# adityabalu/DiffNet

Hardware: AMD Instinct MI355X
Metric: elements*gauss_pts/sec (FEM loss+grad) (higher is better)
Workload: dtype f32; 1 GPU; 2-D Poisson energy loss + gradient wrt u, Q1, 512^2 nodes, 3^2 Gauss pts, batch 64/GPU, nu+f nodal fields, Dirichlet mask on all boundary faces held as one bit per node and sample (a general mask array), fused single pass (BASELINE.json configs[1] mesh); every step evaluates the next of 4 different batches in rotation (nu, f and the mask stream from HBM with non-temporal loads; of the 4 x 67 MB of; batch_per_gpu=64, parallelism=batch-sharded x1, batches_in_rotation=4, mask_format=bits

## Files before the change

### diffnet_amd/csrc/poisson2d_q1_cf.hip

```cpp
#include <cstdlib>
#include <type_traits>

#define DN_NT_STORES 1
#include "poisson_common.h"

namespace dn {

enum : int { CF_NU = 1, CF_F = 2, CF_BC = 8, CF_BC_U8C = 16, CF_BC_PACKED = 32, CF_PK_NB1 = 64, CF_PK_NB2 = 128, CF_UA = 256 };

template <int E>
struct CfRow {
    float u[E + 1], n[E + 1], f[E + 1];
    float g[E + 1];
    float keep[E];
    float keepx;
    BcRaw<E> bc;
    uint32_t m8[2][2];
    uint32_t mb[2];
    uint32_t bx[2];
};

constexpr int CF_W = 4;
constexpr int CF_TS = 128;
constexpr int CF_NSLOT = 64;
constexpr unsigned CF_SPIN_MAX = 1u << 20;

__device__ __forceinline__ unsigned lds_addr(const void* p) { return (unsigned)(uintptr_t)(__attribute__((address_space(3))) const void*)p; }
__device__ __forceinline__ void lds_st(unsigned a, float v) { asm volatile("ds_write_b32 %0, %1" ::"v"(a), "v"(v) : "memory"); }
__device__ __forceinline__ void lds_st(unsigned a, unsigned v) { asm volatile("ds_write_b32 %0, %1" ::"v"(a), "v"(v) : "memory"); }
__device__ __forceinline__ void lds_ld_nowait(float& d, unsigned a) { asm volatile("ds_read_b32 %0, %1" : "=v"(d) : "v"(a) : "memory"); }
__device__ __forceinline__ unsigned lds_ld_u(unsigned a) {
    unsigned d;
    asm volatile("ds_read_b32 %0, %1\n\ts_waitcnt lgkmcnt(0)" : "=v"(d) : "v"(a) : "memory");
    return d;
}
__device__ __forceinline__ float lds_ld(unsigned a) {
    float d;
    asm volatile("ds_read_b32 %0, %1\n\ts_waitcnt lgkmcnt(0)" : "=v"(d) : "v"(a) : "memory");
    return d;
}
template <int N>
__device__ __forceinline__ void lds_wait(float (&v)[N]) {
    if constexpr (N == 5) asm volatile("s_waitcnt lgkmcnt(0)" : "+v"(v[0]), "+v"(v[1]), "+v"(v[2]), "+v"(v[3]), "+v"(v[4])::"memory");
    else if constexpr (N == 4) asm volatile("s_waitcnt lgkmcnt(0)" : "+v"(v[0]), "+v"(v[1]), "+v"(v[2]), "+v"(v[3])::"memory");
    else if constexpr (N == 3) asm volatile("s_waitcnt lgkmcnt(0)" : "+v"(v[0]), "+v"(v[1]), "+v"(v[2])::"memory");
    else if constexpr (N == 2) asm volatile("s_waitcnt lgkmcnt(0)" : "+v"(v[0]), "+v"(v[1])::"memory");
    else { static_assert(N == 1, "lds_wait: 1..5 values"); asm volatile("s_waitcnt lgkmcnt(0)" : "+v"(v[0])::"memory"); }
}

template <int E, bool VEC, int FL, int W>
__global__ void __launch_bounds__(W > 1 ? CF_TS * W : 256, W > 1 ? 4 : 2) poisson2d_q1_cf_kernel(const PoissonParams p) {
    constexpr int NW = E;
    constexpr bool HAS_NU = (FL & CF_NU) != 0, HAS_F = (FL & CF_F) != 0;
    constexpr bool BC_ANY = (FL & (CF_BC | CF_BC_U8C | CF_BC_PACKED)) != 0, BC_U8C = (FL & CF_BC_U8C) != 0, BC_PACKED = (FL & CF_BC_PACKED) != 0;
    constexpr bool UA = (FL & CF_UA) != 0;
    static_assert(!UA || (E == 4 && VEC && W == 1), "CF_UA: four elements per thread, vector accesses, one strip per workgroup");
    const int T = W > 1 ? CF_TS : (int)blockDim.x;
    const int sub = W > 1 ? __builtin_amdgcn_readfirstlane((int)threadIdx.x / CF_TS) : 0;
    const int tid = W > 1 ? (int)threadIdx.x - sub * CF_TS : (int)threadIdx.x;
    const int chunk = blockIdx.x, strip = W > 1 ? (int)blockIdx.y * W + sub : selected_strip(p, (int)blockIdx.y), b = blockIdx.z;
    const bool active = W == 1 || strip < p.nstrips;
    const bool chain_dn = W > 1 && sub > 0;
    const bool chain_up = W > 1 && sub + 1 < W && strip + 1 < p.nstrips;
    const int q = chunk * (T - 1) + tid;
    const int ex0 = q * E;
    const int x0 = ex0;
    const bool col_owner = !(chunk > 0 && tid == 0);
    const bool lastcol = UA && x0 + NW == p.nx - 1;
    const int64_t nps = (int64_t)p.nx * p.ny;
    const SampleBases sb = sample_bases(p, b, nps);
    const int R = p.rows_per_strip;
    const int sb0 = strip * R, sc0 = min(sb0 + R, p.nely);
    const int ey_begin = (sb0 > 0 && !chain_dn) ? sb0 - 1 : sb0;
    const int ey_end = sc0;
    const int r_from = sb0;
    const int e_from = sb0, e_until = p.nely;
    const bool top_row = sc0 == p.nely;

    __shared__ float xch[2][256];
    __shared__ double red[W > 1 ? 4 * W : 8];
    __shared__ int last_flag;
    constexpr int CW = W > 1 ? W : 2, SEAM_WORDS = 6 * (E + 1);
    __shared__ float cf_edge[W > 1 ? W : 1][W > 1 ? CF_NSLOT : 1];
    __shared__ unsigned cf_xflag[W > 1 ? W : 1];
    __shared__ float cf_seam[CW - 1][W > 1 ? SEAM_WORDS : 1][W > 1 ? CF_TS : 1];
    __shared__ unsigned cf_sflag[CW - 1][2][2];
    const int lane = tid & 63, wv = __builtin_amdgcn_readfirstlane(tid >> 6);
    unsigned seq = 0u;
    if constexpr (W > 1) {
        static_assert(CF_TS == 128, "two waves per sub-strip");
        if (threadIdx.x < (unsigned)W) cf_xflag[threadIdx.x] = 0u;
        if (threadIdx.x < 4u * (W - 1)) (&cf_sflag[0][0][0])[threadIdx.x] = 0u;
        __syncthreads();
    }
    if ((blockIdx.x | blockIdx.y | blockIdx.z) == 0u) fold_prev_sums(p, (int)threadIdx.x, (int)blockDim.x, red);
    float spin_poison = 0.f;
    auto spin_until = [&](const unsigned* flag, unsigned want) {
        const unsigned fa = lds_addr(flag);
        const unsigned lim = p.spin_limit > 0 ? (unsigned)p.spin_limit : CF_SPIN_MAX;
        unsigned n = 0;
        for (; n < lim; ++n) {
            if ((unsigned)__builtin_amdgcn_readfirstlane((int)lds_ld_u(fa)) >= want) break;
            __builtin_amdgcn_s_sleep(1);
        }
        if (n == lim) spin_poison = __builtin_nanf("");
    };

    const bool has_mask[2] = {sb.mask[0] != nullptr, sb.mask[1] != nullptr};
    const uint8_t* mask8[2];
    mask8[0] = reinterpret_cast<const uint8_t*>(has_mask[0] ? sb.mask[0] : sb.mask[1]);
    mask8[1] = reinterpret_cast<const uint8_t*>(has_mask[1] ? sb.mask[1] : sb.mask[0]);

    constexpr unsigned NBITS = (1u << (NW + 1)) - 1u;
    constexpr int NB = !BC_PACKED ? 0 : ((FL & CF_PK_NB2) ? 2 : ((FL & CF_PK_NB1) ? 1 : 0));
    const bool isbits[2] = {p.bc[0].kind == DN_MASK_BITS, p.bc[1].kind == DN_MASK_BITS};
    const unsigned bsel[2] = {isbits[0] ? NBITS : 0u, isbits[1] ? NBITS : 0u};
    const int src0 = (NB == 2 || isbits[0]) ? 0 : 1;
    const uint32_t* bptr[2] = {reinterpret_cast<const uint32_t*>(sb.mask[src0]), reinterpret_cast<const uint32_t*>(sb.mask[1])};
    const unsigned brow[2] = {(unsigned)p.bc[src0].row_bytes / 4u, (unsigned)p.bc[1].row_bytes / 4u};
    unsigned bw0[2], bw1[2];
#pragma unroll
    for (int j = 0; j < 2; ++j) {
        const int rw = max((int)brow[j], 1);
        bw0[j] = (unsigned)min(x0 >> 5, rw - 1);
        bw1[j] = (unsigned)min((x0 >> 5) + 1, rw - 1);
    }
    const unsigned bsh = (unsigned)x0 & 31u;
    unsigned boxx[2] = {0u, 0u};
#pragma unroll
    for (int k = 0; k < 2; ++k) {
        const int faces = p.bc[k].kind == DN_MASK_BOX ? p.bc[k].box_faces : 0;
#pragma unroll
        for (int n = 0; n <= NW; ++n) {
            const bool on = ((faces & DN_FACE_XLO) && x0 + n == 0) || ((faces & DN_FACE_XHI) && x0 + n == p.nx - 1);
            boxx[k] |= on ? (1u << n) : 0u;
        }
    }
    const int ylo[2] = {(p.bc[0].kind == DN_MASK_BOX && (p.bc[0].box_faces & DN_FACE_YLO)) ? 0 : -1,
                        (p.bc[1].kind == DN_MASK_BOX && (p.bc[1].box_faces & DN_FACE_YLO)) ? 0 : -1};
    const int yhi[2] = {(p.bc[0].kind == DN_MASK_BOX && (p.bc[0].box_faces & DN_FACE_YHI)) ? p.ny - 1 : -1,
                        (p.bc[1].kind == DN_MASK_BOX && (p.bc[1].box_faces & DN_FACE_YHI)) ? p.ny - 1 : -1};
    auto packed_issue = [&](int yc, CfRow<E>& r) {
#pragma unroll
        for (int j = 0; j < NB; ++j) {
            const unsigned ro = (unsigned)yc * brow[j];
            const uint32_t w0 = ld_at<uint32_t>(bptr[j], ro + bw0[j]), w1 = ld_at<uint32_t>(bptr[j], ro + bw1[j]);
            r.mb[j] = __builtin_amdgcn_alignbit(w1, w0, bsh);
        }
#pragma unroll
        for (int k = 0; k < 2; ++k) r.bx[k] = (yc == ylo[k] || yc == yhi[k]) ? NBITS : boxx[k];
    };

    auto row_issue = [&](int yr, CfRow<E>& r) {
        const int yp = min(yr, p.ny - 1);
        const unsigned rowoff = (unsigned)yp * (unsigned)p.nx;
        load_seg<NW, VEC>(sb.u, rowoff, x0, p.nx, r.u);
        if constexpr (HAS_NU) load_seg_stream<NW, VEC>(sb.nu, rowoff, x0, p.nx, r.n);
        if constexpr (HAS_F) load_seg_stream<NW, VEC>(sb.f, rowoff, x0, p.nx, r.f);
        if constexpr (BC_PACKED) {
            packed_issue(yp, r);
        } else if constexpr (BC_U8C) {
#pragma unroll
            for (int k = 0; k < 2; ++k) {
                if (has_mask[k]) {
                    uint8_t t[NW + 1];
                    load_seg_stream<NW, VEC>(mask8[k], rowoff, x0, p.nx, t);
                    uint32_t w = 0u;
#pragma unroll
                    for (int n = 0; n < NW; ++n) w |= (uint32_t)t[n] << (8 * n);
                    r.m8[k][0] = w;
                    r.m8[k][1] = t[NW];
                }
            }
        } else if constexpr (BC_ANY) {
            bc_issue<NW, VEC>(p, sb, rowoff, x0, r.bc);
        }
    };
    auto row_bc = [&](CfRow<E>& r) {
#pragma unroll
        for (int n = 0; n < NW; ++n) r.keep[n] = 1.f;
        if constexpr (UA) r.keepx = 1.f;
        if constexpr (BC_PACKED) {
            unsigned b0 = r.bx[0], b1 = r.bx[1];
            if constexpr (NB == 2) { b0 |= r.mb[0] & bsel[0]; b1 |= r.mb[1] & bsel[1]; }
            if constexpr (NB == 1) { b0 |= r.mb[0] & bsel[0]; b1 |= r.mb[0] & bsel[1]; }
            const float v0 = p.bc[0].value, v1 = p.bc[1].value;
#pragma unroll
            for (int n = 0; n <= NW; ++n) {
                r.u[n] = (b0 & (1u << n)) ? v0 : r.u[n];
                r.u[n] = (b1 & (1u << n)) ? v1 : r.u[n];
                if (n < NW) r.keep[n] = ((b0 | b1) & (1u << n)) ? 0.f : 1.f;
            }
            if constexpr (UA) r.keepx = ((b0 | b1) & (1u << NW)) ? 0.f : 1.f;
        } else if constexpr (BC_U8C) {
#pragma unroll
            for (int k = 0; k < 2; ++k) {
                if (has_mask[k]) {
                    const float val = p.bc[k].value;
#pragma unroll
                    for (int n = 0; n <= NW; ++n) {
                        const bool set = has_mask[k] && (n < NW ? ((r.m8[k][0] >> (8 * n)) & 0xffu) != 0u : r.m8[k][1] != 0u);
                        r.u[n] = set ? val : r.u[n];
                        if (n < NW) r.keep[n] = set ? 0.f : r.keep[n];
                        else if constexpr (UA) r.keepx = set ? 0.f : r.keepx;
                    }
                }
            }
        } else if constexpr (BC_ANY) {
            if constexpr (UA) {
                float k5[NW + 1];
                bc_apply_all<NW>(p, sb, r.bc, r.u, k5);
#pragma unroll
                for (int n = 0; n < NW; ++n) r.keep[n] = k5[n];
                r.keepx = k5[NW];
            } else {
                bc_apply<NW>(p, sb, r.bc, r.u, r.keep);
            }
        }
    };

    float e1_acc = 0.f, e2_acc = 0.f, sq_acc = 0.f;
    int par = 0;

    float pend_v[NW];
    unsigned pend_row = 0u;
    bool pend_st = false;
    float pend_x = 0.f;
    auto flush_store = [&]() {
        if (pend_st) store_seg<NW, VEC>(sb.out, pend_row, x0, p.nx, pend_v);
        if constexpr (UA) {
            if (pend_st && lastcol) st_at<float>(sb.out, pend_row + (unsigned)(p.nx - 1), pend_x);
        }
        pend_st = false;
    };
    auto emit_row = [&](const float (&o)[NW + 1], const float (&keep)[NW], int yr, bool owned_row, float keepx = 1.f) {
        float left;
        if constexpr (W > 1) {
            const float up = __shfl_up(o[NW], 1, 64);
            const unsigned ea = lds_addr(&cf_edge[sub][seq & (CF_NSLOT - 1)]);
            float edge = 0.f;
            if (wv == 0) {
                if (lane == 63) { lds_st(ea, o[NW]); lds_st(lds_addr(&cf_xflag[sub]), seq + 1u); }
            } else {
                spin_until(&cf_xflag[sub], seq + 1u);
                edge = lds_ld(ea);
            }
            left = lane > 0 ? up : edge;
            ++seq;
        } else {
            xch[par][tid] = o[NW];
            asm volatile("s_waitcnt lgkmcnt(0)\n\ts_barrier" ::: "memory");
            left = (tid > 0) ? xch[par][tid - 1] : 0.f;
            par ^= 1;
        }
        const bool st = owned_row && col_owner && (!UA || x0 + NW <= p.nx - 1);
#pragma unroll
        for (int n = 0; n < NW; ++n) {
            const float t = (o[n] + (n == 0 ? left : 0.f)) * keep[n];
            sq_acc = st ? fmaf(t, t, sq_acc) : sq_acc;
            pend_v[n] = t * p.out_scale;
            if constexpr (W > 1) pend_v[n] += spin_poison;
        }
        if constexpr (UA) {
            const float t = o[NW] * keepx;
            sq_acc = (st && lastcol) ? fmaf(t, t, sq_acc) : sq_acc;
            pend_x = t * p.out_scale;
        }
        pend_row = (unsigned)yr * (unsigned)p.nx;
        pend_st = st && sb.out != nullptr;
        flush_store();
    };

    const float mx0 = p.T.mxs[0], mx1 = p.T.mxs[1], mx2 = p.T.mxs[2], mx3 = p.T.mxs[3];
    const float my0 = p.T.m[0], my1 = p.T.m[1], my2 = p.T.m[2], my3 = p.T.m[3];
    const float k0 = p.T.q1c[0], k1 = p.T.q1c[1], h0 = p.T.q1c[2], h1 = p.T.q1c[3], nb = -p.T.beta;

    constexpr bool FMASS = HAS_F && (FL & CF_BC) == 0;
    const float cx00 = p.T.q1mx[0], cx01 = p.T.q1mx[1], cx11 = p.T.q1mx[2], cy00 = p.T.q1my[0], cy01 = p.T.q1my[1], cy11 = p.T.q1my[2];
    auto fstage = [&](CfRow<E>& r) {
        if constexpr (FMASS) {
#pragma unroll
            for (int n = 0; n <= NW; ++n) r.g[n] = 0.f;
#pragma unroll
            for (int e = 0; e < E; ++e) {
                if (ex0 + e < p.nelx) {
                    r.g[e] = fmaf(cx01, r.f[e + 1], fmaf(cx00, r.f[e], r.g[e]));
                    r.g[e + 1] = fmaf(cx11, r.f[e + 1], cx01 * r.f[e]);
                }
            }
        }
    };

    auto layer = [&](auto fresh, int ey, const CfRow<E>& L, CfRow<E>& U, const float (&cin)[NW + 1], float (&cout)[NW + 1]) {
        const bool own_layer = ey >= e_from && ey <= e_until;
        const float cnt = (own_layer && col_owner) ? 1.f : 0.f;
        if constexpr (decltype(fresh)::value) { row_bc(U); fstage(U); }
        float o[NW + 1], le1 = 0.f, le2 = 0.f;
#pragma unroll
        for (int n = 0; n <= NW; ++n) { o[n] = cin[n]; cout[n] = 0.f; }
        if constexpr (FMASS) {
#pragma unroll
            for (int n = 0; n <= NW; ++n) {
                const float tlo = fmaf(cy01, U.g[n], cy00 * L.g[n]), tup = fmaf(cy11, U.g[n], cy01 * L.g[n]);
                o[n] = fmaf(nb, tlo, o[n]);
                cout[n] = nb * tup;
                le2 = fmaf(U.u[n], tup, fmaf(L.u[n], tlo, le2));
            }
        }
#pragma unroll
        for (int e = 0; e < E; ++e) {
            if (ex0 + e < p.nelx) {
                const float U0 = L.u[e], UX = L.u[e + 1] - L.u[e], UY = U.u[e] - L.u[e], UXY = (U.u[e + 1] - U.u[e]) - UX;
                float P = mx0, Q = 0.f, Pp = my0, Qp = 0.f;
                if constexpr (HAS_NU) {
                    const float N0 = L.n[e], NX = L.n[e + 1] - N0, NY = U.n[e] - N0, NXY = (U.n[e + 1] - U.n[e]) - NX;
                    P = fmaf(mx1, NX, mx0 * N0);
                    Q = fmaf(mx1, NXY, mx0 * NY);
                    Pp = fmaf(my1, NY, my0 * N0);
                    Qp = fmaf(my1, NXY, my0 * NX);
                }
                const float A0 = fmaf(Q, my1, P * my0), A1 = fmaf(Q, my2, P * my1), A2 = fmaf(Q, my3, P * my2);
                const float B0 = fmaf(Qp, mx1, Pp * mx0), B1 = fmaf(Qp, mx2, Pp * mx1), B2 = fmaf(Qp, mx3, Pp * mx2);
                const float tX0 = fmaf(UXY, A1, UX * A0), tX1 = fmaf(UXY, A2, UX * A1);
                const float tY0 = fmaf(UXY, B1, UY * B0), tY1 = fmaf(UXY, B2, UY * B1);
                le1 += fmaf(h1, fmaf(UXY, tY1, UY * tY0), h0 * fmaf(UXY, tX1, UX * tX0));
                float cU0 = 0.f, cUX = k0 * tX0, cUY = k1 * tY0, cUXY = fmaf(k0, tX1, k1 * tY1);
                if constexpr (HAS_F && !FMASS) {
                    const float F0 = L.f[e], FX = L.f[e + 1] - F0, FY = U.f[e] - F0, FXY = (U.f[e + 1] - U.f[e]) - FX;
                    const float S0 = fmaf(mx1, FX, mx0 * F0), S1 = fmaf(mx1, FXY, mx0 * FY);
                    const float T0 = fmaf(mx2, FX, mx1 * F0), T1 = fmaf(mx2, FXY, mx1 * FY);
                    const float L0 = fmaf(my1, S1, my0 * S0), LX = fmaf(my1, T1, my0 * T0);
                    const float LY = fmaf(my2, S1, my1 * S0), LXY = fmaf(my2, T1, my1 * T0);
                    le2 += fmaf(LXY, UXY, fmaf(LY, UY, fmaf(LX, UX, L0 * U0)));
                    cU0 = nb * L0;
                    cUX = fmaf(nb, LX, cUX);
                    cUY = fmaf(nb, LY, cUY);
                    cUXY = fmaf(nb, LXY, cUXY);
                }
                const float g01 = cUX - cUXY, g10 = cUY - cUXY;
                o[e] += (cU0 - cUX) - g10;
                o[e + 1] += g01;
                cout[e] += g10;
                cout[e + 1] += cUXY;
            }
        }
        e1_acc = fmaf(cnt, le1, e1_acc);
        e2_acc = fmaf(cnt, le2, e2_acc);
        if (W > 1 && chain_dn && ey == sb0) {
            const unsigned s0 = lds_addr(&cf_seam[W > 1 ? sub - 1 : 0][0][tid]);
#pragma unroll
            for (int n = 0; n <= NW; ++n) lds_st(s0 + (4 * NW + 4 + n) * CF_TS * 4, o[n]);
#pragma unroll
            for (int n = 0; n < NW; ++n) lds_st(s0 + (5 * NW + 5 + n) * CF_TS * 4, L.keep[n]);
        } else {
            emit_row(o, L.keep, ey, ey >= r_from, L.keepx);
        }
    };
    auto publish_row = [&](const CfRow<E>& r) {
        const unsigned s0 = lds_addr(&cf_seam[W > 1 ? sub - 1 : 0][0][tid]);
#pragma unroll
        for (int n = 0; n <= NW; ++n) {
            lds_st(s0 + n * CF_TS * 4, r.u[n]);
            if constexpr (HAS_NU) lds_st(s0 + (NW + 1 + n) * CF_TS * 4, r.n[n]);
            if constexpr (FMASS) lds_st(s0 + (2 * NW + 2 + n) * CF_TS * 4, r.g[n]);
            else if constexpr (HAS_F) lds_st(s0 + (2 * NW + 2 + n) * CF_TS * 4, r.f[n]);
        }
        if (lane == 0) lds_st(lds_addr(&cf_sflag[W > 1 ? sub - 1 : 0][0][wv]), 1u);
    };
    auto fetch_row = [&](CfRow<E>& r) {
        spin_until(&cf_sflag[sub][0][wv], 1u);
        const unsigned s0 = lds_addr(&cf_seam[sub][0][tid]);
#pragma unroll
        for (int n = 0; n <= NW; ++n) lds_ld_nowait(r.u[n], s0 + n * CF_TS * 4);
        lds_wait(r.u);
        if constexpr (HAS_NU) {
#pragma unroll
            for (int n = 0; n <= NW; ++n) lds_ld_nowait(r.n[n], s0 + (NW + 1 + n) * CF_TS * 4);
            lds_wait(r.n);
        }
        if constexpr (FMASS) {
#pragma unroll
            for (int n = 0; n <= NW; ++n) lds_ld_nowait(r.g[n], s0 + (2 * NW + 2 + n) * CF_TS * 4);
            lds_wait(r.g);
        } else if constexpr (HAS_F) {
#pragma unroll
            for (int n = 0; n <= NW; ++n) lds_ld_nowait(r.f[n], s0 + (2 * NW + 2 + n) * CF_TS * 4);
            lds_wait(r.f);
        }
    };
    auto publish_carry = [&](const float (&c)[NW + 1]) {
        const unsigned s0 = lds_addr(&cf_seam[sub][0][tid]);
#pragma unroll
        for (int n = 0; n <= NW; ++n) lds_st(s0 + (3 * NW + 3 + n) * CF_TS * 4, c[n]);
        if (lane == 0) lds_st(lds_addr(&cf_sflag[sub][1][wv]), 1u);
    };

    auto set_prio = [&](int e) {
        switch (((ey_end - e) >> 1) & 3) {
            case 0: __builtin_amdgcn_s_setprio(0); break;
            case 1: __builtin_amdgcn_s_setprio(1); break;
            case 2: __builtin_amdgcn_s_setprio(2); break;
            default: __builtin_amdgcn_s_setprio(3); break;
        }
    };

    constexpr std::true_type FRESH{};
    constexpr std::false_type LANDED{};
    if (active) {
    CfRow<E> RA, RB;
    float carryA[NW + 1], carryB[NW + 1];
#pragma unroll
    for (int n = 0; n <= NW; ++n) carryA[n] = carryB[n] = 0.f;
    row_issue(ey_begin, RA);
    row_bc(RA);
    fstage(RA);
    if constexpr (W > 1) {
        if (chain_dn) publish_row(RA);
    }
    int ey = ey_begin;
    bool odd = false;
    const int n_main = chain_up ? ey_end - 1 : ey_end;
    for (; ey + 1 < n_main; ey += 2) {
        set_prio(ey);
        row_issue(ey + 1, RB);
        layer(FRESH, ey, RA, RB, carryA, carryB);
        row_issue(ey + 2, RA);
        layer(FRESH, ey + 1, RB, RA, carryB, carryA);
    }
    if (ey < n_main) {
        set_prio(ey);
        row_issue(ey + 1, RB);
        layer(FRESH, ey, RA, RB, carryA, carryB);
        odd = true;
        ++ey;
    }
    if constexpr (W > 1) {
        if (chain_up) {
            __builtin_amdgcn_s_setprio(0);
            if (odd) { fetch_row(RA); layer(LANDED, ey, RB, RA, carryB, carryA); publish_carry(carryA); }
            else { fetch_row(RB); layer(LANDED, ey, RA, RB, carryA, carryB); publish_carry(carryB); }
        }
    }
    if (top_row) {
        float o[NW + 1], keep[NW];
#pragma unroll
        for (int n = 0; n <= NW; ++n) o[n] = odd ? carryB[n] : carryA[n];
#pragma unroll
        for (int n = 0; n < NW; ++n) keep[n] = odd ? RB.keep[n] : RA.keep[n];
        emit_row(o, keep, p.ny - 1, true, odd ? RB.keepx : RA.keepx);
        flush_store();
    }
    if constexpr (W > 1) {
        if (chain_dn) {
            spin_until(&cf_sflag[sub - 1][1][wv], 1u);
            const unsigned s0 = lds_addr(&cf_seam[sub - 1][0][tid]);
            float o[NW + 1], cy[NW + 1], keep[NW];
#pragma unroll
            for (int n = 0; n <= NW; ++n) lds_ld_nowait(o[n], s0 + (4 * NW + 4 + n) * CF_TS * 4);
            lds_wait(o);
#pragma unroll
            for (int n = 0; n <= NW; ++n) lds_ld_nowait(cy[n], s0 + (3 * NW + 3 + n) * CF_TS * 4);
            lds_wait(cy);
#pragma unroll
            for (int n = 0; n < NW; ++n) lds_ld_nowait(keep[n], s0 + (5 * NW + 5 + n) * CF_TS * 4);
            lds_wait(keep);
#pragma unroll
            for (int n = 0; n <= NW; ++n) o[n] += cy[n];
            emit_row(o, keep, sb0, true);
            flush_store();
        }
    }
    }

    if constexpr (W > 1) {
        e1_acc += spin_poison;
        sq_acc += spin_poison;
        if (spin_poison != spin_poison && p.counter != nullptr && (threadIdx.x & 63u) == 0u) atomicOr(p.counter + DN_WS_ERRWORD, 1u);
    }
    if (p.want_sums) finish_sums(p, e1_acc, e2_acc, sq_acc, (int)threadIdx.x, (int)blockDim.x, red, &last_flag);
}

template <int E, bool VEC, int FL>
static void cf_launch_one(const PoissonParams& pp, const Geom2D& g, int batch, hipStream_t s) {
    if constexpr (E == 4 && VEC && (FL & CF_UA) == 0) {
        if (g.W == CF_W) {
            hipLaunchKernelGGL((poisson2d_q1_cf_kernel<E, VEC, FL, CF_W>), dim3(g.chunks, (g.strips + CF_W - 1) / CF_W, batch),
                               dim3(CF_TS * CF_W), 0, s, pp);
            return;
        }
    }
    hipLaunchKernelGGL((poisson2d_q1_cf_kernel<E, VEC, FL, 1>), dim3(g.chunks, g.strips, batch), dim3(g.T), 0, s, pp);
}

template <int E, bool VEC, int UAF = 0>
static void cf_launch_flags(const PoissonParams& pp, const Geom2D& g, int batch, hipStream_t s) {
    const bool any = pp.bc[0].kind >= 0 || pp.bc[1].kind >= 0;
    bool u8c = any, packed = false;
    for (int k = 0; k < 2; ++k) {
        if (pp.bc[k].kind >= 0 && (!pp.bc[k].mask_is_u8 || pp.bc[k].field)) u8c = false;
        if (pp.bc[k].kind == DN_MASK_BITS || pp.bc[k].kind == DN_MASK_BOX) packed = true;
    }
    const int nbits = (pp.bc[0].kind == DN_MASK_BITS) + (pp.bc[1].kind == DN_MASK_BITS);
    const int nf = (pp.nu ? CF_NU : 0) | (pp.f ? CF_F : 0);
#define DN_CF(FLAGS)                                                                         \
    (!any ? cf_launch_one<E, VEC, (FLAGS) | UAF>(pp, g, batch, s)                                  \
          : packed ? (nbits == 2 ? cf_launch_one<E, VEC, (FLAGS) | UAF | CF_BC_PACKED | CF_PK_NB2>(pp, g, batch, s)          \
                     : nbits == 1 ? cf_launch_one<E, VEC, (FLAGS) | UAF | CF_BC_PACKED | CF_PK_NB1>(pp, g, batch, s)        \
                                  : cf_launch_one<E, VEC, (FLAGS) | UAF | CF_BC_PACKED>(pp, g, batch, s))                   \
          : u8c ? cf_launch_one<E, VEC, (FLAGS) | UAF | CF_BC_U8C>(pp, g, batch, s)                \
                : cf_launch_one<E, VEC, (FLAGS) | UAF | CF_BC>(pp, g, batch, s))
    switch (nf) {
        case 0: DN_CF(0); break;
        case CF_NU: DN_CF(CF_NU); break;
        case CF_F: DN_CF(CF_F); break;
        default: DN_CF(CF_NU | CF_F); break;
    }
#undef DN_CF
}

int poisson2d_q1_cf_chain() { return CF_W; }

int launch_poisson2d_q1_cf(const PoissonParams& pp, const Geom2D& g, int batch, bool vec, hipStream_t s) {
    if (g.W > 1 && !(g.W == poisson2d_q1_cf_chain() && g.E == 4 && vec && g.T == CF_TS && g.R + 3 <= CF_NSLOT)) return DN_E_BADARG;
    if (g.ua) {
        if (g.E != 4 || g.W != 1 || (pp.nx & 3) != 1 || pp.nx < 9) return DN_E_BADARG;
        cf_launch_flags<4, true, CF_UA>(pp, g, batch, s);
        return 0;
    }
    if (g.E == 4 && vec) { cf_launch_flags<4, true>(pp, g, batch, s); return 0; }
    if (g.E == 2 && vec) { cf_launch_flags<2, true>(pp, g, batch, s); return 0; }
    if (g.E == 2) { cf_launch_flags<2, false>(pp, g, batch, s); return 0; }
    return DN_E_UNSUPPORTED;
}

}
```

### diffnet_amd/csrc/poisson_elem.h

```cpp
#pragma once
#include "dn_common.h"

namespace dn {

typedef float v2f __attribute__((ext_vector_type(2)));
__device__ __forceinline__ float vfma(float a, float b, float c) { return fmaf(a, b, c); }
__device__ __forceinline__ v2f vfma(v2f a, v2f b, v2f c) { return __builtin_elementwise_fma(a, b, c); }
__device__ __forceinline__ v2f vfma(float a, v2f b, v2f c) { return __builtin_elementwise_fma((v2f)(a), b, c); }

struct ElemTab {
    float b[4][4];
    float dx[4][4];
    float dy[4][4];
    float dz[4][4];
    float w[4];
    float wx[4];
    float w2[4][4];
    float hs[3];
    float ahs[3];
    float alpha, beta, c;
    float m[4];
    float mxs[4];
    float kx[3][4];
    float q1c[4];
    float wb[4];
    float kap[3];
    float hs2[3];
    float m01, m12;
    float esc;
    float nbw;
    float q1mx[3], q1my[3];
};

template <int P, int NGP, bool FGP>
__device__ __forceinline__ void elem2d(const ElemTab& T, const float (&u)[P + 1][P + 1], const float (&nu)[P + 1][P + 1],
                                       const float (&f)[P + 1][P + 1], const float* fg, float (&g)[P + 1][P + 1],
                                       float& e1, float& e2) {
    constexpr int NB = P + 1;
    float a1 = 0.f, a2 = 0.f;
    static_assert(P >= 2, "Q1 elements run through the marching kernels (q1_layer_2d / q1_layer_3d)");
#pragma unroll
    for (int jb = 0; jb < NB; ++jb)
#pragma unroll
        for (int ib = 0; ib < NB; ++ib) g[jb][ib] = 0.f;
#pragma unroll
    for (int ig = 0; ig < NGP; ++ig) {
        float tv[NB], td[NB], tn[NB], tf[NB], rv[NB], rd[NB];
#pragma unroll
        for (int jb = 0; jb < NB; ++jb) {
            float a = 0.f, d = 0.f, n = 0.f, q = 0.f;
#pragma unroll
            for (int ib = 0; ib < NB; ++ib) {
                a = fmaf(T.b[ig][ib], u[jb][ib], a);
                d = fmaf(T.dx[ig][ib], u[jb][ib], d);
                n = fmaf(T.b[ig][ib], nu[jb][ib], n);
                if constexpr (!FGP) q = fmaf(T.b[ig][ib], f[jb][ib], q);
            }
            tv[jb] = a; td[jb] = d; tn[jb] = n; tf[jb] = q; rv[jb] = 0.f; rd[jb] = 0.f;
        }
#pragma unroll
        for (int jg = 0; jg < NGP; ++jg) {
            float val = 0.f, ux = 0.f, uy = 0.f, nuv = 0.f, fv = 0.f;
#pragma unroll
            for (int jb = 0; jb < NB; ++jb) {
                val = fmaf(T.b[jg][jb], tv[jb], val);
                ux = fmaf(T.b[jg][jb], td[jb], ux);
                uy = fmaf(T.dy[jg][jb], tv[jb], uy);
                nuv = fmaf(T.b[jg][jb], tn[jb], nuv);
                if constexpr (!FGP) fv = fmaf(T.b[jg][jb], tf[jb], fv);
            }
            if constexpr (FGP) fv = fg[jg * NGP + ig];
            const float Wn = T.w2[jg][ig] * nuv, Wf = T.w2[jg][ig] * fv;
            a1 = fmaf(Wn, ux * ux + uy * uy, a1);
            a2 = fmaf(Wf, val, a2);
            const float qx = T.alpha * Wn * ux, qy = T.alpha * Wn * uy, qv = -T.beta * Wf;
#pragma unroll
            for (int jb = 0; jb < NB; ++jb) {
                rv[jb] = fmaf(T.b[jg][jb], qv, rv[jb]);
                rv[jb] = fmaf(T.dy[jg][jb], qy, rv[jb]);
                rd[jb] = fmaf(T.b[jg][jb], qx, rd[jb]);
            }
        }
#pragma unroll
        for (int jb = 0; jb < NB; ++jb)
// ... 12 lines not shown
                                            const float DX1, const float (&TN0)[NGP], const float (&TN1)[NGP],
                                            const float (&TF0)[NGP], const float (&TF1)[NGP], const float* fg,
                                            float (&ct0)[NGP], float (&ct1)[NGP], float& cdx0, float& cdx1, float& e1,
                                            float& e2) {
    float a1x = 0.f, a1y = 0.f, a2 = 0.f;
    float S0 = 0.f, S1 = 0.f, dyn[NGP];
#pragma unroll
    for (int i = 0; i < NGP; ++i) {
        dyn[i] = TN1[i] - TN0[i];
        S0 = fmaf(T.wx[i], TN0[i], S0);
        S1 = fmaf(T.wx[i], dyn[i], S1);
    }
    const float ddx = DX1 - DX0;
    float c1s = 0.f, css = 0.f;
#pragma unroll
    for (int jg = 0; jg < NGP; ++jg) {
        const float r = fmaf(T.b[jg][1], ddx, DX0);
        const float t = fmaf(T.b[jg][1], S1, S0) * r;
        a1x = fmaf(T.w[jg] * t, r, a1x);
        const float cx = T.w[jg] * t;
        css += cx;
        c1s = fmaf(T.b[jg][1], cx, c1s);
    }
    const float kx = T.q1c[0];
    cdx1 = kx * c1s;
    cdx0 = kx * css - cdx1;
    const float nb = -T.beta, ky = T.q1c[1];
#pragma unroll
    for (int ig = 0; ig < NGP; ++ig) {
        const float dyv = TU1[ig] - TU0[ig];
        const float t = fmaf(T.kx[1][ig], dyn[ig], T.kx[0][ig] * TN0[ig]) * dyv;
        a1y = fmaf(t, dyv, a1y);
        float cs, c1;
        if constexpr (FGP) {
            cs = 0.f; c1 = 0.f;
#pragma unroll
            for (int jg = 0; jg < NGP; ++jg) {
                const float wf = T.w2[jg][ig] * fg[jg * NGP + ig];
                cs += wf;
                c1 = fmaf(T.b[jg][1], wf, c1);
            }
        } else {
            const float dyf = TF1[ig] - TF0[ig];
            cs = fmaf(T.kx[1][ig], dyf, T.kx[0][ig] * TF0[ig]);
            c1 = fmaf(T.kx[2][ig], dyf, T.kx[1][ig] * TF0[ig]);
        }
        a2 = fmaf(cs, TU0[ig], a2);
        a2 = fmaf(c1, dyv, a2);
        ct1[ig] = fmaf(nb, c1, ky * t);
        ct0[ig] = fmaf(nb, cs, -ct1[ig]);
    }
    e1 = fmaf(T.q1c[2], a1x, T.q1c[3] * a1y);
    e2 = a2;
}

template <int NGP, bool FGP>
__device__ __forceinline__ void q1_layer_3d(const ElemTab& T, const float (&LU)[NGP][NGP], const float (&UU)[NGP][NGP],
                                            const float (&LX)[NGP], const float (&UX)[NGP], const float (&LY)[NGP],
                                            const float (&UY)[NGP], const float (&LN)[NGP][NGP], const float (&UN)[NGP][NGP],
                                            const float (&LF)[NGP][NGP], const float (&UF)[NGP][NGP], const float* fg,
                                            float (&cUL)[NGP][NGP], float (&cUU)[NGP][NGP], float (&cXL)[NGP], float (&cXU)[NGP],
                                            float (&cYL)[NGP], float (&cYU)[NGP], float& e1, float& e2) {
    float a1 = 0.f, a2 = 0.f;
    float A0[NGP], A1[NGP], B0[NGP], B1[NGP];
#pragma unroll
    for (int i = 0; i < NGP; ++i) A0[i] = A1[i] = B0[i] = B1[i] = 0.f;
    const float nb = -T.beta;
#pragma unroll
    for (int jg = 0; jg < NGP; ++jg) {
#pragma unroll
        for (int ig = 0; ig < NGP; ++ig) {
            const float w2 = T.w2[jg][ig];
            const float dzu = UU[jg][ig] - LU[jg][ig];
            const float uz = T.hs[2] * dzu;
            const float dzn = UN[jg][ig] - LN[jg][ig];
            const float wn0 = w2 * LN[jg][ig], wn1 = w2 * dzn;
            A0[jg] += wn0; A1[jg] += wn1; B0[ig] += wn0; B1[ig] += wn1;
            const float Qz = fmaf(T.m[1], wn1, T.m[0] * wn0);
            const float qzu = Qz * uz;
            a1 = fmaf(qzu, uz, a1);
            const float cz = T.ahs[2] * qzu;
            float cs, c1;
            if constexpr (FGP) {
                cs = 0.f; c1 = 0.f;
#pragma unroll
                for (int kg = 0; kg < NGP; ++kg) {
                    const float wf = T.w[kg] * w2 * fg[(kg * NGP + jg) * NGP + ig];
                    cs += wf;
                    c1 = fmaf(T.b[kg][1], wf, c1);
                }
            } else {
                const float dzf = UF[jg][ig] - LF[jg][ig];
                const float wf0 = w2 * LF[jg][ig], wf1 = w2 * dzf;
                cs = fmaf(T.m[1], wf1, T.m[0] * wf0);
                c1 = fmaf(T.m[2], wf1, T.m[1] * wf0);
            }
            a2 = fmaf(cs, LU[jg][ig], a2);
            a2 = fmaf(c1, dzu, a2);
            cUU[jg][ig] = fmaf(nb, c1, cz);
            cUL[jg][ig] = fmaf(nb, cs, -cUU[jg][ig]);
        }
    }
#pragma unroll
    for (int jg = 0; jg < NGP; ++jg) {
        const float dv = UX[jg] - LX[jg];
        float sx = 0.f, tx = 0.f;
// ... 125 lines not shown
```

### diffnet_amd/csrc/poisson_fused.hip

```cpp
#include <algorithm>
#include <cmath>
#include <cstdio>
#include <cstdlib>

#include "poisson_common.h"

namespace dn {

template <int P, int NGP, int E, bool VEC, bool FGP>
__global__ void __launch_bounds__(256) poisson2d_kernel(const PoissonParams p) {
    constexpr int NB = P + 1;
    constexpr int NW = E * P;
    const int T = blockDim.x;
    const int tid = threadIdx.x;
    const int chunk = blockIdx.x, strip = selected_strip(p, (int)blockIdx.y), b = blockIdx.z;
    const int q = chunk * (T - 1) + tid;
    const int ex0 = q * E;
    const int x0 = ex0 * P;
    const bool col_owner = !(chunk > 0 && tid == 0);
    const int64_t nps = (int64_t)p.nx * p.ny;
    const unsigned eps = (unsigned)(p.nelx * p.nely);
    const SampleBases sb = sample_bases(p, b, nps);
    const float* fgp = FGP ? p.fgp + (p.f_batched ? (int64_t)b * eps * (NGP * NGP) : 0) : nullptr;
    const int R = p.rows_per_strip;
// ... 398 lines not shown
        const bool present = d.mask_kind == DN_MASK_BOX ? d.box_faces != 0 : d.mask != nullptr;
        if (present && (d.mask_kind == DN_MASK_BITS || d.mask_kind == DN_MASK_BOX)) {
            packed_bc = true;
            if (d.field) return DN_E_BADARG;
            if (d.mask_kind == DN_MASK_BITS && d.row_words < (m->nx + 31) / 32) return DN_E_BADARG;
        }
    }
    if (packed_bc && m->nsd == 3) {
        for (int k = 0; k < 2; ++k)
            if (a->bc[k].mask_kind == DN_MASK_BITS) return DN_E_UNSUPPORTED;
        if (gen3d || !q1n2_ok(m, a)) return DN_E_UNSUPPORTED;
    } else if (packed_bc) {
        if (m->nsd != 2 || P != 1 || a->f_gp || config(CFG_Q1_RULE_KERNEL) != nullptr) return DN_E_UNSUPPORTED;
        for (int k = 0; k < 2; ++k) {
            const dn_dirichlet& d = a->bc[k];
            if (d.mask && (d.mask_kind == DN_MASK_F32 || d.mask_kind == DN_MASK_U8)) return DN_E_UNSUPPORTED;
        }
    }
    const bool want_red = a->energy || a->sumsq || a->energy_f32;
    auto vec_ok = [&](int NW) { return poisson_vec_ok(m, a, NW); };
    const bool allow_e4 = vec_ok(4);
    const long long nwg = gen3d ? 1 : num_workgroups(m, allow_e4);
    if (nwg >= (1ll << 31)) return DN_E_UNSUPPORTED;
    if (!gen3d && want_red && (!a->workspace || a->workspace_bytes < DN_WS_HEADER + (int64_t)(2 * sizeof(double)) * nwg)) return DN_E_WORKSPACE;
    if ((int64_t)m->nx * m->ny * (m->nsd == 3 ? m->nz : 1) >= (1ll << 30)) return DN_E_UNSUPPORTED;

    PoissonParams pp;
    for (int i = 0; i < 4; ++i) {
        for (int j = 0; j < 4; ++j) {
            pp.T.b[i][j] = m->basis[i][j];
            pp.T.dx[i][j] = m->dbasis[i][j] * m->scale[0];
            pp.T.dy[i][j] = m->dbasis[i][j] * m->scale[1];
            pp.T.dz[i][j] = m->dbasis[i][j] * m->scale[2];
        }
        pp.T.w[i] = m->gpw[i];
        pp.T.wx[i] = m->gpw[i] * a->wscale;
    }
    for (int i = 0; i < 4; ++i)
        for (int j = 0; j < 4; ++j) pp.T.w2[i][j] = pp.T.w[i] * pp.T.wx[j];
    for (int d = 0; d < 3; ++d) {
        pp.T.hs[d] = 0.5f * m->scale[d];
        pp.T.ahs[d] = a->alpha * pp.T.hs[d];
    }
    pp.T.q1c[0] = a->alpha * pp.T.hs[0] * pp.T.hs[0]; pp.T.q1c[1] = a->alpha * pp.T.hs[1] * pp.T.hs[1];
    pp.T.q1c[2] = pp.T.hs[0] * pp.T.hs[0];            pp.T.q1c[3] = pp.T.hs[1] * pp.T.hs[1];
    {
        double mm[4] = {0.0, 0.0, 0.0, 0.0};
        for (int g = 0; g < m->ngp; ++g) {
            const double bb = m->basis[g][1];
            mm[0] += m->gpw[g]; mm[1] += m->gpw[g] * bb; mm[2] += m->gpw[g] * bb * bb; mm[3] += m->gpw[g] * bb * bb * bb;
        }
        pp.T.q1my[0] = (float)(mm[0] - 2.0 * mm[1] + mm[2]); pp.T.q1my[1] = (float)(mm[1] - mm[2]); pp.T.q1my[2] = (float)mm[2];
        for (int r = 0; r < 3; ++r) pp.T.q1mx[r] = (float)((double)(r == 0 ? mm[0] - 2.0 * mm[1] + mm[2] : (r == 1 ? mm[1] - mm[2] : mm[2])) * (double)a->wscale);
        for (int r = 0; r < 4; ++r) {
            pp.T.m[r] = (float)mm[r];
            pp.T.mxs[r] = (float)(mm[r] * (double)a->wscale);
            if (r < 3)
                for (int g = 0; g < 4; ++g) pp.T.kx[r][g] = (float)(mm[r] * (double)m->gpw[g] * (double)a->wscale);
        }
    }
    for (int g = 0; g < 4; ++g) pp.T.wb[g] = m->gpw[g] * m->basis[g][1];
    for (int d = 0; d < 3; ++d) {
        pp.T.hs2[d] = pp.T.hs[d] * pp.T.hs[d];
        pp.T.kap[d] = a->alpha * a->wscale * pp.T.hs2[d];
    }
    pp.T.m01 = pp.T.m[0] - pp.T.m[1]; pp.T.m12 = pp.T.m[1] - pp.T.m[2];
    pp.T.esc = a->wscale; pp.T.nbw = -a->beta * a->wscale;
    pp.T.alpha = a->alpha; pp.T.beta = a->beta; pp.T.c = a->c;
    pp.u = a->u; pp.nu = a->nu; pp.f = a->f; pp.fgp = a->f_gp;
    pp.nu_batched = a->nu_batched; pp.f_batched = a->f_batched;
    pp.f_is_load = (a->f_is_load && a->f) ? 1 : 0;
    if (pp.f_is_load && !(m->nsd == 3 && !gen3d && q1n2_ok(m, a))) return DN_E_UNSUPPORTED;
    for (int k = 0; k < 2; ++k) {
        const dn_dirichlet& d = a->bc[k];
        const bool present = d.mask_kind == DN_MASK_BOX ? d.box_faces != 0 : d.mask != nullptr;
        pp.bc[k].mask = d.mask_kind == DN_MASK_BOX ? nullptr : d.mask; pp.bc[k].field = d.field; pp.bc[k].value = d.value;
        pp.bc[k].mask_is_u8 = d.mask_kind == DN_MASK_U8; pp.bc[k].mask_batched = d.mask_batched;
        pp.bc[k].field_batched = d.field_batched;
        pp.bc[k].kind = present ? d.mask_kind : -1;
        pp.bc[k].box_faces = d.box_faces; pp.bc[k].row_bytes = 4 * d.row_words;
    }
    pp.out_scale = a->out_scale; pp.out = a->out;
    pp.counter = reinterpret_cast<unsigned*>(a->workspace);
    pp.part_energy = a->workspace ? reinterpret_cast<double*>(reinterpret_cast<char*>(a->workspace) + DN_WS_HEADER) : nullptr;
    pp.part_sumsq = pp.part_energy ? pp.part_energy + nwg : nullptr;
    pp.energy = a->energy; pp.sumsq = a->sumsq;
    pp.energy_f32 = a->energy_f32; pp.energy_scale = a->energy_scale;
    pp.nx = m->nx; pp.ny = m->ny; pp.nz = m->nsd == 3 ? m->nz : 1;
    pp.nelx = (m->nx - 1) / P; pp.nely = (m->ny - 1) / P; pp.nelz = m->nsd == 3 ? (m->nz - 1) / P : 1;
    pp.want_sums = want_red ? 1 : 0;
    pp.spin_limit = config(CFG_HANDOVER_SPIN_LIMIT) ? std::atoi(config(CFG_HANDOVER_SPIN_LIMIT)) : 0;
    hipStream_t s = reinterpret_cast<hipStream_t>(stream);
    pp.fold_n = 0;
    if (a->fold_prev) {
        const dn_poisson_args* q = a->fold_prev;
        if (gen3d || !q->defer_sums || !q->workspace || !(q->energy || q->sumsq || q->energy_f32)) return DN_E_BADARG;
        if (q->accumulate_sums && !(q->energy && q->sumsq)) return DN_E_BADARG;
        if (q->workspace == a->workspace && want_red) return DN_E_BADARG;
        const long long qn = launched_workgroups(m, q), qstride = num_workgroups(m, poisson_vec_ok(m, q, 4));
        if (q->workspace_bytes < DN_WS_HEADER + (int64_t)(2 * sizeof(double)) * qstride || qn > qstride) return DN_E_WORKSPACE;
        const bool cf2d = m->nsd == 2 && P == 1 && a->f_gp == nullptr && config(CFG_Q1_RULE_KERNEL) == nullptr;
        if (!cf2d && !(m->nsd == 3 && q1n2_ok(m, a))) return DN_E_UNSUPPORTED;
        pp.fold_pe = reinterpret_cast<const double*>(reinterpret_cast<const char*>(q->workspace) + DN_WS_HEADER);
        pp.fold_ps = pp.fold_pe + qstride;
        pp.fold_n = (int)qn;
        pp.fold_energy = q->energy; pp.fold_sumsq = q->sumsq; pp.fold_energy_f32 = q->energy_f32;
// ... 92 lines not shown
```

Baseline: 2487 billion elements*gauss_pts/s.

## Restructure Q1 element math into row-staged factors and specialize single-mask path

Reformulates the per-element Q1 energy/gradient using per-row precomputed differences (du) and nu projections (pn) plus column differences V and S, so shared terms between adjacent rows and columns are computed once instead of per element. New host-side moment coefficients (q1xm, q1ym, q1px, q1sy) support the factored form. Adds a CF_ONE specialization for the case where only one boundary condition slot is active, which skips loading and combining the second mask. This trades some extra per-row registers for fewer ALU operations per element, and carries a risk of small floating-point differences from the regrouped arithmetic.

```diff
diff --git a/diffnet_amd/csrc/poisson2d_q1_cf.hip b/diffnet_amd/csrc/poisson2d_q1_cf.hip
--- a/diffnet_amd/csrc/poisson2d_q1_cf.hip
+++ b/diffnet_amd/csrc/poisson2d_q1_cf.hip
@@ -6,12 +6,13 @@
 
 namespace dn {
 
-enum : int { CF_NU = 1, CF_F = 2, CF_BC = 8, CF_BC_U8C = 16, CF_BC_PACKED = 32, CF_PK_NB1 = 64, CF_PK_NB2 = 128, CF_UA = 256 };
+enum : int { CF_NU = 1, CF_F = 2, CF_BC = 8, CF_BC_U8C = 16, CF_BC_PACKED = 32, CF_PK_NB1 = 64, CF_PK_NB2 = 128, CF_UA = 256, CF_ONE = 512 };
 
 template <int E>
 struct CfRow {
     float u[E + 1], n[E + 1], f[E + 1];
     float g[E + 1];
+    float du[E], pn[E];
     float keep[E];
     float keepx;
     BcRaw<E> bc;
@@ -53,7 +54,8 @@
     constexpr int NW = E;
     constexpr bool HAS_NU = (FL & CF_NU) != 0, HAS_F = (FL & CF_F) != 0;
     constexpr bool BC_ANY = (FL & (CF_BC | CF_BC_U8C | CF_BC_PACKED)) != 0, BC_U8C = (FL & CF_BC_U8C) != 0, BC_PACKED = (FL & CF_BC_PACKED) != 0;
-    constexpr bool UA = (FL & CF_UA) != 0;
+    constexpr bool UA = (FL & CF_UA) != 0, ONE = (FL & CF_ONE) != 0;
+    static_assert(!ONE || ((BC_PACKED || BC_U8C) && (FL & CF_PK_NB2) == 0), "CF_ONE: one packed or uint8-constant condition");
     static_assert(!UA || (E == 4 && VEC && W == 1), "CF_UA: four elements per thread, vector accesses, one strip per workgroup");
     const int T = W > 1 ? CF_TS : (int)blockDim.x;
     const int sub = W > 1 ? __builtin_amdgcn_readfirstlane((int)threadIdx.x / CF_TS) : 0;
@@ -116,6 +118,7 @@
     const bool isbits[2] = {p.bc[0].kind == DN_MASK_BITS, p.bc[1].kind == DN_MASK_BITS};
     const unsigned bsel[2] = {isbits[0] ? NBITS : 0u, isbits[1] ? NBITS : 0u};
     const int src0 = (NB == 2 || isbits[0]) ? 0 : 1;
+    const int kone = p.bc[0].kind >= 0 ? 0 : 1;
     const uint32_t* bptr[2] = {reinterpret_cast<const uint32_t*>(sb.mask[src0]), reinterpret_cast<const uint32_t*>(sb.mask[1])};
     const unsigned brow[2] = {(unsigned)p.bc[src0].row_bytes / 4u, (unsigned)p.bc[1].row_bytes / 4u};
     unsigned bw0[2], bw1[2];
@@ -147,8 +150,12 @@
             const uint32_t w0 = ld_at<uint32_t>(bptr[j], ro + bw0[j]), w1 = ld_at<uint32_t>(bptr[j], ro + bw1[j]);
             r.mb[j] = __builtin_amdgcn_alignbit(w1, w0, bsh);
         }
-#pragma unroll
-        for (int k = 0; k < 2; ++k) r.bx[k] = (yc == ylo[k] || yc == yhi[k]) ? NBITS : boxx[k];
+        if constexpr (ONE) {
+            if constexpr (NB == 0) r.bx[0] = (yc == (kone ? ylo[1] : ylo[0]) || yc == (kone ? yhi[1] : yhi[0])) ? NBITS : (kone ? boxx[1] : boxx[0]);
+        } else {
+#pragma unroll
+            for (int k = 0; k < 2; ++k) r.bx[k] = (yc == ylo[k] || yc == yhi[k]) ? NBITS : boxx[k];
+        }
     };
 
     auto row_issue = [&](int yr, CfRow<E>& r) {
@@ -159,6 +166,14 @@
         if constexpr (HAS_F) load_seg_stream<NW, VEC>(sb.f, rowoff, x0, p.nx, r.f);
         if constexpr (BC_PACKED) {
             packed_issue(yp, r);
+        } else if constexpr (BC_U8C && ONE) {
+            uint8_t t[NW + 1];
+            load_seg_stream<NW, VEC>(mask8[0], rowoff, x0, p.nx, t);
+            uint32_t w = 0u;
+#pragma unroll
+            for (int n = 0; n < NW; ++n) w |= (uint32_t)t[n] << (8 * n);
+            r.m8[0][0] = w;
+            r.m8[0][1] = t[NW];
         } else if constexpr (BC_U8C) {
 #pragma unroll
             for (int k = 0; k < 2; ++k) {
@@ -180,7 +195,20 @@
 #pragma unroll
         for (int n = 0; n < NW; ++n) r.keep[n] = 1.f;
         if constexpr (UA) r.keepx = 1.f;
-        if constexpr (BC_PACKED) {
+        if constexpr ((BC_PACKED || BC_U8C) && ONE) {
+            const float v = kone ? p.bc[1].value : p.bc[0].value;
+            unsigned b = 0u;
+            if constexpr (BC_PACKED) b = NB == 1 ? r.mb[0] : r.bx[0];
+#pragma unroll
+            for (int n = 0; n <= NW; ++n) {
+                bool set;
+                if constexpr (BC_PACKED) set = (b & (1u << n)) != 0u;
+                else set = n < NW ? ((r.m8[0][0] >> (8 * n)) & 0xffu) != 0u : r.m8[0][1] != 0u;
+                r.u[n] = set ? v : r.u[n];
+                if (n < NW) r.keep[n] = set ? 0.f : 1.f;
+                else if constexpr (UA) r.keepx = set ? 0.f : 1.f;
+            }
+        } else if constexpr (BC_PACKED) {
             unsigned b0 = r.bx[0], b1 = r.bx[1];
             if constexpr (NB == 2) { b0 |= r.mb[0] & bsel[0]; b1 |= r.mb[1] & bsel[1]; }
             if constexpr (NB == 1) { b0 |= r.mb[0] & bsel[0]; b1 |= r.mb[0] & bsel[1]; }
@@ -274,9 +302,13 @@
     const float mx0 = p.T.mxs[0], mx1 = p.T.mxs[1], mx2 = p.T.mxs[2], mx3 = p.T.mxs[3];
     const float my0 = p.T.m[0], my1 = p.T.m[1], my2 = p.T.m[2], my3 = p.T.m[3];
     const float k0 = p.T.q1c[0], k1 = p.T.q1c[1], h0 = p.T.q1c[2], h1 = p.T.q1c[3], nb = -p.T.beta;
-
-    constexpr bool FMASS = HAS_F && (FL & CF_BC) == 0;
+    constexpr bool ROWSTAGED = (FL & CF_BC) == 0, STAGE_DU = W == 1;
+    const float xm[4] = {p.T.q1xm[0], p.T.q1xm[1], p.T.q1xm[2], p.T.q1xm[3]}, ym[4] = {p.T.q1ym[0], p.T.q1ym[1], p.T.q1ym[2], p.T.q1ym[3]};
+    const float px0 = p.T.q1px[0], px1 = p.T.q1px[1], sy0 = p.T.q1sy[0], sy1 = p.T.q1sy[1];
+
+    constexpr bool FMASS = HAS_F && ROWSTAGED;
     const float cx00 = p.T.q1mx[0], cx01 = p.T.q1mx[1], cx11 = p.T.q1mx[2], cy00 = p.T.q1my[0], cy01 = p.T.q1my[1], cy11 = p.T.q1my[2];
+    const float alpha = p.T.alpha;
     auto fstage = [&](CfRow<E>& r) {
         if constexpr (FMASS) {
 #pragma unroll
@@ -291,10 +323,25 @@
         }
     };
 
+    auto sstage = [&](CfRow<E>& r) {
+        if constexpr (ROWSTAGED) {
+#pragma unroll
+            for (int e = 0; e < E; ++e) {
+                if constexpr (HAS_NU) {
+                    q1cf_stage(px0, px1, r.u[e], r.u[e + 1], r.n[e], r.n[e + 1], r.du[e], r.pn[e]);
+                } else {
+                    r.du[e] = r.u[e + 1] - r.u[e];
+                    r.pn[e] = mx0;
+                }
+            }
+        }
+    };
+
     auto layer = [&](auto fresh, int ey, const CfRow<E>& L, CfRow<E>& U, const float (&cin)[NW + 1], float (&cout)[NW + 1]) {
         const bool own_layer = ey >= e_from && ey <= e_until;
         const float cnt = (own_layer && col_owner) ? 1.f : 0.f;
         if constexpr (decltype(fresh)::value) { row_bc(U); fstage(U); }
+        sstage(U);
         float o[NW + 1], le1 = 0.f, le2 = 0.f;
 #pragma unroll
         for (int n = 0; n <= NW; ++n) { o[n] = cin[n]; cout[n] = 0.f; }
@@ -307,41 +354,57 @@
                 le2 = fmaf(U.u[n], tup, fmaf(L.u[n], tlo, le2));
             }
         }
-#pragma unroll
-        for (int e = 0; e < E; ++e) {
-            if (ex0 + e < p.nelx) {
-                const float U0 = L.u[e], UX = L.u[e + 1] - L.u[e], UY = U.u[e] - L.u[e], UXY = (U.u[e + 1] - U.u[e]) - UX;
-                float P = mx0, Q = 0.f, Pp = my0, Qp = 0.f;
-                if constexpr (HAS_NU) {
-                    const float N0 = L.n[e], NX = L.n[e + 1] - N0, NY = U.n[e] - N0, NXY = (U.n[e + 1] - U.n[e]) - NX;
-                    P = fmaf(mx1, NX, mx0 * N0);
-                    Q = fmaf(mx1, NXY, mx0 * NY);
-                    Pp = fmaf(my1, NY, my0 * N0);
-                    Qp = fmaf(my1, NXY, my0 * NX);
+        if constexpr (ROWSTAGED) {
+            float V[NW + 1], S[NW + 1];
+#pragma unroll
+            for (int n = 0; n <= NW; ++n) {
+                V[n] = U.u[n] - L.u[n];
+                S[n] = HAS_NU ? fmaf(sy1, U.n[n], sy0 * L.n[n]) : my0;
+            }
+#pragma unroll
+            for (int e = 0; e < E; ++e) {
+                if (ex0 + e < p.nelx) {
+                    const float a = STAGE_DU ? L.du[e] : L.u[e + 1] - L.u[e], b = STAGE_DU ? U.du[e] : U.u[e + 1] - U.u[e];
+                    q1cf_elem(xm, ym, a, b, L.pn[e], U.pn[e], V[e], V[e + 1], S[e], S[e + 1], alpha, o[e], o[e + 1], cout[e], cout[e + 1], le1);
                 }
-                const float A0 = fmaf(Q, my1, P * my0), A1 = fmaf(Q, my2, P * my1), A2 = fmaf(Q, my3, P * my2);
-                const float B0 = fmaf(Qp, mx1, Pp * mx0), B1 = fmaf(Qp, mx2, Pp * mx1), B2 = fmaf(Qp, mx3, Pp * mx2);
-                const float tX0 = fmaf(UXY, A1, UX * A0), tX1 = fmaf(UXY, A2, UX * A1);
-                const float tY0 = fmaf(UXY, B1, UY * B0), tY1 = fmaf(UXY, B2, UY * B1);
-                le1 += fmaf(h1, fmaf(UXY, tY1, UY * tY0), h0 * fmaf(UXY, tX1, UX * tX0));
-                float cU0 = 0.f, cUX = k0 * tX0, cUY = k1 * tY0, cUXY = fmaf(k0, tX1, k1 * tY1);
-                if constexpr (HAS_F && !FMASS) {
-                    const float F0 = L.f[e], FX = L.f[e + 1] - F0, FY = U.f[e] - F0, FXY = (U.f[e + 1] - U.f[e]) - FX;
-                    const float S0 = fmaf(mx1, FX, mx0 * F0), S1 = fmaf(mx1, FXY, mx0 * FY);
-                    const float T0 = fmaf(mx2, FX, mx1 * F0), T1 = fmaf(mx2, FXY, mx1 * FY);
-                    const float L0 = fmaf(my1, S1, my0 * S0), LX = fmaf(my1, T1, my0 * T0);
-                    const float LY = fmaf(my2, S1, my1 * S0), LXY = fmaf(my2, T1, my1 * T0);
-                    le2 += fmaf(LXY, UXY, fmaf(LY, UY, fmaf(LX, UX, L0 * U0)));
-                    cU0 = nb * L0;
-                    cUX = fmaf(nb, LX, cUX);
-                    cUY = fmaf(nb, LY, cUY);
-                    cUXY = fmaf(nb, LXY, cUXY);
+            }
+        } else {
+#pragma unroll
+            for (int e = 0; e < E; ++e) {
+                if (ex0 + e < p.nelx) {
+                    const float U0 = L.u[e], UX = L.u[e + 1] - L.u[e], UY = U.u[e] - L.u[e], UXY = (U.u[e + 1] - U.u[e]) - UX;
+                    float P = mx0, Q = 0.f, Pp = my0, Qp = 0.f;
+                    if constexpr (HAS_NU) {
+                        const float N0 = L.n[e], NX = L.n[e + 1] - N0, NY = U.n[e] - N0, NXY = (U.n[e + 1] - U.n[e]) - NX;
+                        P = fmaf(mx1, NX, mx0 * N0);
+                        Q = fmaf(mx1, NXY, mx0 * NY);
+                        Pp = fmaf(my1, NY, my0 * N0);
+                        Qp = fmaf(my1, NXY, my0 * NX);
+                    }
+                    const float A0 = fmaf(Q, my1, P * my0), A1 = fmaf(Q, my2, P * my1), A2 = fmaf(Q, my3, P * my2);
+                    const float B0 = fmaf(Qp, mx1, Pp * mx0), B1 = fmaf(Qp, mx2, Pp * mx1), B2 = fmaf(Qp, mx3, Pp * mx2);
+                    const float tX0 = fmaf(UXY, A1, UX * A0), tX1 = fmaf(UXY, A2, UX * A1);
+                    const float tY0 = fmaf(UXY, B1, UY * B0), tY1 = fmaf(UXY, B2, UY * B1);
+                    le1 += fmaf(h1, fmaf(UXY, tY1, UY * tY0), h0 * fmaf(UXY, tX1, UX * tX0));
+                    float cU0 = 0.f, cUX = k0 * tX0, cUY = k1 * tY0, cUXY = fmaf(k0, tX1, k1 * tY1);
+                    if constexpr (HAS_F) {
+                        const float F0 = L.f[e], FX = L.f[e + 1] - F0, FY = U.f[e] - F0, FXY = (U.f[e + 1] - U.f[e]) - FX;
+                        const float S0 = fmaf(mx1, FX, mx0 * F0), S1 = fmaf(mx1, FXY, mx0 * FY);
+                        const float T0 = fmaf(mx2, FX, mx1 * F0), T1 = fmaf(mx2, FXY, mx1 * FY);
+                        const float L0 = fmaf(my1, S1, my0 * S0), LX = fmaf(my1, T1, my0 * T0);
+                        const float LY = fmaf(my2, S1, my1 * S0), LXY = fmaf(my2, T1, my1 * T0);
+                        le2 += fmaf(LXY, UXY, fmaf(LY, UY, fmaf(LX, UX, L0 * U0)));
+                        cU0 = nb * L0;
+                        cUX = fmaf(nb, LX, cUX);
+                        cUY = fmaf(nb, LY, cUY);
+                        cUXY = fmaf(nb, LXY, cUXY);
+                    }
+                    const float g01 = cUX - cUXY, g10 = cUY - cUXY;
+                    o[e] += (cU0 - cUX) - g10;
+                    o[e + 1] += g01;
+                    cout[e] += g10;
+                    cout[e + 1] += cUXY;
                 }
-                const float g01 = cUX - cUXY, g10 = cUY - cUXY;
-                o[e] += (cU0 - cUX) - g10;
-                o[e + 1] += g01;
-                cout[e] += g10;
-                cout[e + 1] += cUXY;
             }
         }
         e1_acc = fmaf(cnt, le1, e1_acc);
@@ -414,6 +477,7 @@
     row_issue(ey_begin, RA);
     row_bc(RA);
     fstage(RA);
+    sstage(RA);
     if constexpr (W > 1) {
         if (chain_dn) publish_row(RA);
     }
@@ -501,13 +565,17 @@
         if (pp.bc[k].kind == DN_MASK_BITS || pp.bc[k].kind == DN_MASK_BOX) packed = true;
     }
     const int nbits = (pp.bc[0].kind == DN_MASK_BITS) + (pp.bc[1].kind == DN_MASK_BITS);
+    const bool one = (pp.bc[0].kind >= 0) != (pp.bc[1].kind >= 0);
     const int nf = (pp.nu ? CF_NU : 0) | (pp.f ? CF_F : 0);
 #define DN_CF(FLAGS)                                                                         \
     (!any ? cf_launch_one<E, VEC, (FLAGS) | UAF>(pp, g, batch, s)                                  \
           : packed ? (nbits == 2 ? cf_launch_one<E, VEC, (FLAGS) | UAF | CF_BC_PACKED | CF_PK_NB2>(pp, g, batch, s)          \
-                     : nbits == 1 ? cf_launch_one<E, VEC, (FLAGS) | UAF | CF_BC_PACKED | CF_PK_NB1>(pp, g, batch, s)        \
-                                  : cf_launch_one<E, VEC, (FLAGS) | UAF | CF_BC_PACKED>(pp, g, batch, s))                   \
-          : u8c ? cf_launch_one<E, VEC, (FLAGS) | UAF | CF_BC_U8C>(pp, g, batch, s)                \
+                     : nbits == 1 ? (one ? cf_launch_one<E, VEC, (FLAGS) | UAF | CF_BC_PACKED | CF_PK_NB1 | CF_ONE>(pp, g, batch, s)        \
+                                         : cf_launch_one<E, VEC, (FLAGS) | UAF | CF_BC_PACKED | CF_PK_NB1>(pp, g, batch, s))        \
+                     : one ? cf_launch_one<E, VEC, (FLAGS) | UAF | CF_BC_PACKED | CF_ONE>(pp, g, batch, s)                   \
+                           : cf_launch_one<E, VEC, (FLAGS) | UAF | CF_BC_PACKED>(pp, g, batch, s))                   \
+          : u8c ? (one ? cf_launch_one<E, VEC, (FLAGS) | UAF | CF_BC_U8C | CF_ONE>(pp, g, batch, s)                \
+                       : cf_launch_one<E, VEC, (FLAGS) | UAF | CF_BC_U8C>(pp, g, batch, s))                \
                 : cf_launch_one<E, VEC, (FLAGS) | UAF | CF_BC>(pp, g, batch, s))
     switch (nf) {
         case 0: DN_CF(0); break;
diff --git a/diffnet_amd/csrc/poisson_elem.h b/diffnet_amd/csrc/poisson_elem.h
--- a/diffnet_amd/csrc/poisson_elem.h
+++ b/diffnet_amd/csrc/poisson_elem.h
@@ -30,6 +30,10 @@
     float esc;
     float nbw;
     float q1mx[3], q1my[3];
+    float q1xm[4];
+    float q1ym[4];
+    float q1px[2];
+    float q1sy[2];
 };
 
 template <int P, int NGP, bool FGP>
@@ -148,6 +152,27 @@
     }
     e1 = fmaf(T.q1c[2], a1x, T.q1c[3] * a1y);
     e2 = a2;
+}
+
+__host__ __device__ __forceinline__ void q1cf_stage(const float px0, const float px1, const float u0, const float u1, const float n0, const float n1,
+                                                    float& du, float& pn) {
+    du = u1 - u0;
+    pn = fmaf(px1, n1, px0 * n0);
+}
+
+__host__ __device__ __forceinline__ void q1cf_elem(const float (&xm)[4], const float (&ym)[4], const float a, const float b, const float p,
+                                                   const float q, const float V0, const float V1, const float S0, const float S1,
+                                                   const float alpha, float& gL0, float& gL1, float& gU0, float& gU1, float& e) {
+    const float X0 = fmaf(q, xm[1], p * xm[0]), X1 = fmaf(q, xm[2], p * xm[1]), X2 = fmaf(q, xm[3], p * xm[2]);
+    const float ta = fmaf(b, X1, a * X0), tb = fmaf(b, X2, a * X1);
+    const float Y0 = fmaf(S1, ym[1], S0 * ym[0]), Y1 = fmaf(S1, ym[2], S0 * ym[1]), Y2 = fmaf(S1, ym[3], S0 * ym[2]);
+    const float t0 = fmaf(V1, Y1, V0 * Y0), t1 = fmaf(V1, Y2, V0 * Y1);
+    e = fmaf(b, tb, fmaf(a, ta, e));
+    e = fmaf(V1, t1, fmaf(V0, t0, e));
+    gL0 = fmaf(-alpha, ta + t0, gL0);
+    gL1 = fmaf(alpha, ta - t1, gL1);
+    gU0 = fmaf(alpha, t0 - tb, gU0);
+    gU1 = fmaf(alpha, tb + t1, gU1);
 }
 
 template <int NGP, bool FGP>
diff --git a/diffnet_amd/csrc/poisson_fused.hip b/diffnet_amd/csrc/poisson_fused.hip
--- a/diffnet_amd/csrc/poisson_fused.hip
+++ b/diffnet_amd/csrc/poisson_fused.hip
@@ -474,6 +474,16 @@
         }
         pp.T.q1my[0] = (float)(mm[0] - 2.0 * mm[1] + mm[2]); pp.T.q1my[1] = (float)(mm[1] - mm[2]); pp.T.q1my[2] = (float)mm[2];
         for (int r = 0; r < 3; ++r) pp.T.q1mx[r] = (float)((double)(r == 0 ? mm[0] - 2.0 * mm[1] + mm[2] : (r == 1 ? mm[1] - mm[2] : mm[2])) * (double)a->wscale);
+        {
+            const double rr[4] = {mm[0] - 3.0 * mm[1] + 3.0 * mm[2] - mm[3], mm[1] - 2.0 * mm[2] + mm[3], mm[2] - mm[3], mm[3]};
+            const double hx = 0.5 * (double)m->scale[0], hy = 0.5 * (double)m->scale[1], ws = a->wscale;
+            for (int r = 0; r < 4; ++r) {
+                pp.T.q1xm[r] = (float)(hx * hx * rr[r]);
+                pp.T.q1ym[r] = (float)(hy * hy * ws * rr[r]);
+            }
+            pp.T.q1px[0] = (float)((mm[0] - mm[1]) * ws); pp.T.q1px[1] = (float)(mm[1] * ws);
+            pp.T.q1sy[0] = (float)(mm[0] - mm[1]);        pp.T.q1sy[1] = (float)mm[1];
+        }
         for (int r = 0; r < 4; ++r) {
             pp.T.m[r] = (float)mm[r];
             pp.T.mxs[r] = (float)(mm[r] * (double)a->wscale);
```

Result: faster. 2648 billion elements*gauss_pts/s, median of 6 (+6.5%).
